# HaokunChen245/FedDAT

Measured on AMD Instinct MI355X. Metric: VQA samples/sec, ViLT-B/32 dual-adapter local step, higher is better.
Workload: dtype fp16; 1 GPU; configs[1] with fp16 operands (BASELINE.json's configs[1] string says bf16: same operand width and MFMA rate; the bf16 step is in other_operand_format with --full): ViLT-B/32 FedDAT, 1 client per MI355X, fp16 MFMA operands (dynamic loss scale, GradScaler semantics on the device, initial 2^14), fp32 accumulate / masters, batch=32/client, 384x384 synthetic + 40-token questions, MKD on; batch_per_client=32, seq_len=185, clients=1, hip_graph=True, ranks=1, hetero_steps=False

## Files before the change

### feddat_amd/csrc/head_tail.hip

```cpp
#include "common.hip.h"

namespace {

constexpr int HT_JT = 4;
constexpr int HT_NW = 8;
constexpr int HT_U = 3;

struct HtJob {
    const float* A; long sa_i, sa_k;
    const float* B; long sb_k, sb_j;
    int I, J, K;
    int mode;
    float alpha;
    const float* alpha_dev;
    const float* bias_j;
    float* out; long ldo;
    float* colsum;
    int pro;
    const float* pro_a;
    const float* pro_b;
    float pro_eps;
    float* stats_out;
    int epi;
    const float* aux; long ld_aux;
    int itiles, jblocks;
    int avec, bvec;
    int jt;
};
struct HtLaunch {
    HtJob job[2];
    int blocks0;
};

template <bool AV, bool BV, int JT>
__device__ __forceinline__ void ht_mainloop(const HtJob& p, const float* ap, const float* yp, const float* const (&bp)[JT],
                                            const bool iv, const bool (&jv)[JT], const int g, const float mean,
                                            const float rstd, const int c_first, const int c_step, f32x4 (&acc)[JT],
                                            float& asum) {
    const int nchunk = (p.K + 15) >> 4;
    for (int c0 = c_first; c0 < nchunk; c0 += c_step * HT_U) {
        f32x4 a[HT_U], y[HT_U], ga[HT_U], be[HT_U], b[HT_U][JT];
#pragma unroll
        for (int u = 0; u < HT_U; ++u) {
            const int k0 = (c0 + c_step * u) * 16 + 4 * g;
            const bool in = k0 < p.K;
            const int kc = in ? k0 : 0;
#pragma unroll
            for (int e = 0; e < 4; ++e) {
                const int ke = min(k0 + e, p.K - 1);
                if (!AV) a[u][e] = ap[(size_t)ke * p.sa_k];
                if (!AV && p.pro == FEDDAT_HT_PRO_TANH_BWD) y[u][e] = yp[(size_t)ke * p.sa_k];
            }
            if (AV) {
                a[u] = *reinterpret_cast<const f32x4*>(ap + kc);
                if (p.pro == FEDDAT_HT_PRO_TANH_BWD) y[u] = *reinterpret_cast<const f32x4*>(yp + kc);
            }
            if (p.pro == FEDDAT_HT_PRO_LN) {
                ga[u] = *reinterpret_cast<const f32x4*>(p.pro_a + kc);
                be[u] = *reinterpret_cast<const f32x4*>(p.pro_b + kc);
            }
#pragma unroll
            for (int t = 0; t < JT; ++t) {
                if (BV) {
                    b[u][t] = *reinterpret_cast<const f32x4*>(bp[t] + kc);
                } else {
#pragma unroll
                    for (int e = 0; e < 4; ++e) b[u][t][e] = bp[t][(size_t)min(k0 + e, p.K - 1) * p.sb_k];
                }
            }
        }
#pragma unroll
        for (int u = 0; u < HT_U; ++u) {
            const int k0 = (c0 + c_step * u) * 16 + 4 * g;
#pragma unroll
            for (int e = 0; e < 4; ++e) {
                const bool kv = (k0 + e) < p.K && (c0 + c_step * u) < nchunk;
                float av = a[u][e];
                if (p.pro == FEDDAT_HT_PRO_LN) av = (av - mean) * rstd * ga[u][e] + be[u][e];
                if (p.pro == FEDDAT_HT_PRO_TANH_BWD) av = av * (1.f - y[u][e] * y[u][e]);
                av = (iv && kv) ? av : 0.f;
                asum += av;
#pragma unroll
                for (int t = 0; t < JT; ++t) acc[t] = mfma16x4_f32(av, (jv[t] && kv) ? b[u][t][e] : 0.f, acc[t]);
            }
        }
    }
}

template <int JT>
__device__ __forceinline__ void ht_body(const HtJob& p, const int wid, float* ht_smem) {
    float (*red)[64][HT_JT * 4 + 4] = reinterpret_cast<float (*)[64][HT_JT * 4 + 4]>(ht_smem);
    float (*srow)[2] = reinterpret_cast<float (*)[2]>(ht_smem + (HT_NW - 1) * 64 * (HT_JT * 4 + 4));
    const int lane = threadIdx.x & 63, wave = threadIdx.x >> 6;
    const int itile = wid / p.jblocks, jb = wid - itile * p.jblocks;
    const int i16 = lane & 15, g = lane >> 4;
    const int i = itile * 16 + i16;
    const bool iv = i < p.I;
    const float* ap = p.A + (size_t)(iv ? i : 0) * p.sa_i;
    const float* yp = p.pro == FEDDAT_HT_PRO_TANH_BWD ? p.pro_a + (size_t)(iv ? i : 0) * p.sa_i : nullptr;

    float mean = 0.f, rstd = 0.f;
    if (p.pro == FEDDAT_HT_PRO_LN) {
        for (int rl = wave; rl < 16; rl += HT_NW) {
            const int r = itile * 16 + rl;
            if (r >= p.I) continue;
            const float* xr = p.A + (size_t)r * p.sa_i;
            const int nc = p.K >> 2;
            f32x4 v[8];
            float s = 0.f;
#pragma unroll
            for (int c = 0; c < 8; ++c) {
                const int q4 = lane + c * 64;
                if (q4 < nc) {
                    v[c] = *reinterpret_cast<const f32x4*>(xr + q4 * 4);
                    s += v[c][0] + v[c][1] + v[c][2] + v[c][3];
                }
            }
            const float m = wave_sum(s) / (float)p.K;
            float q = 0.f;
#pragma unroll
            for (int c = 0; c < 8; ++c)
                if (lane + c * 64 < nc)
#pragma unroll
                    for (int e = 0; e < 4; ++e) {
                        const float d = v[c][e] - m;
                        q += d * d;
                    }
            const float rs = rsqrtf(wave_sum(q) / (float)p.K + p.pro_eps);
            if (lane == 0) {
                srow[rl][0] = m;
                srow[rl][1] = rs;
                if (p.stats_out && jb == 0) {
                    p.stats_out[2 * r] = m;
                    p.stats_out[2 * r + 1] = rs;
                }
            }
        }
        __syncthreads();
        mean = srow[i16][0];
        rstd = srow[i16][1];
    }

    const int jgrp = p.mode == 0 ? jb : jb * HT_NW + wave;
    int j[JT];
    bool jv[JT];
    const float* bp[JT];
#pragma unroll
    for (int t = 0; t < JT; ++t) {
        j[t] = (jgrp * JT + t) * 16 + i16;
        jv[t] = j[t] < p.J;
        bp[t] = p.B + (size_t)(jv[t] ? j[t] : 0) * p.sb_j;
    }
    f32x4 acc[JT];
#pragma unroll
    for (int t = 0; t < JT; ++t) acc[t] = f32x4{0.f, 0.f, 0.f, 0.f};
    float asum = 0.f;
    const int c_first = p.mode == 0 ? wave : 0, c_step = p.mode == 0 ? HT_NW : 1;
    if (p.avec && p.bvec) ht_mainloop<true, true, JT>(p, ap, yp, bp, iv, jv, g, mean, rstd, c_first, c_step, acc, asum);
    else if (p.avec) ht_mainloop<true, false, JT>(p, ap, yp, bp, iv, jv, g, mean, rstd, c_first, c_step, acc, asum);
    else if (p.bvec) ht_mainloop<false, true, JT>(p, ap, yp, bp, iv, jv, g, mean, rstd, c_first, c_step, acc, asum);
    else ht_mainloop<false, false, JT>(p, ap, yp, bp, iv, jv, g, mean, rstd, c_first, c_step, acc, asum);
    asum += __shfl_xor(asum, 16, 64);
    asum += __shfl_xor(asum, 32, 64);
    if (p.mode == 0) {
        if (wave > 0) {
            float* dst = red[wave - 1][lane];
#pragma unroll
            for (int t = 0; t < JT; ++t) *reinterpret_cast<f32x4*>(dst + 4 * t) = acc[t];
            dst[JT * 4] = asum;
        }
        __syncthreads();
        if (wave != 0) return;
#pragma unroll 1
        for (int w = 0; w < HT_NW - 1; ++w) {
            const float* src = red[w][lane];
#pragma unroll
            for (int t = 0; t < JT; ++t) acc[t] = acc[t] + *reinterpret_cast<const f32x4*>(src + 4 * t);
            asum += src[JT * 4];
        }
    }
    const float alpha = p.alpha_dev ? p.alpha * *p.alpha_dev : p.alpha;
#pragma unroll
    for (int t = 0; t < JT; ++t) {
        if (!jv[t]) continue;
        const float bj = p.bias_j ? p.bias_j[j[t]] : 0.f;
#pragma unroll
        for (int e = 0; e < 4; ++e) {
            const int io = itile * 16 + 4 * g + e;
            if (io >= p.I) continue;
            float v = alpha * acc[t][e] + bj;
            if (p.epi == FEDDAT_HT_EPI_TANH) v = tanhf(v);
            if (p.epi == FEDDAT_HT_EPI_MUL_DGELU) v *= gelu_grad_f(p.aux[(size_t)io * p.ld_aux + j[t]]);
            p.out[(size_t)io * p.ldo + j[t]] = v;
        }
    }
    if (p.colsum && jgrp == 0 && g == 0 && iv) p.colsum[i] = alpha * asum;
}

__global__ __launch_bounds__(HT_NW * 64) void ht_gemm_kernel(const HtLaunch L) {
    extern __shared__ __attribute__((aligned(16))) float ht_smem[];
    const bool second = (int)blockIdx.x >= L.blocks0;
    const HtJob& p = L.job[second ? 1 : 0];
    const int wid = second ? blockIdx.x - L.blocks0 : blockIdx.x;
    if (p.jt == 1) ht_body<1>(p, wid, ht_smem);
    else ht_body<HT_JT>(p, wid, ht_smem);
}

__global__ __launch_bounds__(256) void ht_ln_gelu_kernel(const float* __restrict__ x, const float* __restrict__ gamma,
                                                         const float* __restrict__ beta, float eps, int rows, int H,
                                                         float* __restrict__ y, float* __restrict__ stats,
                                                         float* __restrict__ gl) {
    const int row = blockIdx.x * 4 + (threadIdx.x >> 6), lane = threadIdx.x & 63;
    if (row >= rows) return;
    const int nc = H >> 2;
    const float* xr = x + (size_t)row * H;
    f32x4 v[8];
    float s = 0.f;
#pragma unroll
    for (int c = 0; c < 8; ++c) {
        const int i = lane + c * 64;
        if (i < nc) {
            v[c] = *reinterpret_cast<const f32x4*>(xr + i * 4);
            s += v[c][0] + v[c][1] + v[c][2] + v[c][3];
        }
    }
    const float mean = wave_sum(s) / (float)H;
    float q = 0.f;
#pragma unroll
    for (int c = 0; c < 8; ++c)
        if (lane + c * 64 < nc)
#pragma unroll
            for (int e = 0; e < 4; ++e) {
                const float d = v[c][e] - mean;
                q += d * d;
            }
    const float rstd = rsqrtf(wave_sum(q) / (float)H + eps);
    if (lane == 0) {
        stats[2 * row] = mean;
        stats[2 * row + 1] = rstd;
    }
#pragma unroll
    for (int c = 0; c < 8; ++c) {
        const int i = lane + c * 64;
        if (i < nc) {
            const f32x4 g4 = *reinterpret_cast<const f32x4*>(gamma + i * 4);
// ... 492 lines not shown
__global__ void single_step_finish_kernel(const SingleFinish s, int* flag, float* scaler_f, int* scaler_i, float growth,
                                          float backoff, int growth_interval) {
    if (blockIdx.x != 0 || threadIdx.x != 0) return;
    const int applied = *flag ? 0 : 1;
    for (int k = 0; k < s.n; ++k) {
        s.state[k][0] += applied;
        s.state[k][1] += applied;
    }
    float scale = scaler_f[0];
    int tracker = scaler_i[0];
    if (!applied) {
        scale = fmaxf(scale * backoff, 6.103515625e-05f);
        tracker = 0;
        scaler_i[1] += 1;
        scaler_i[2] += 1;
    } else {
        tracker += 1;
        if (tracker >= growth_interval) {
            scale = fminf(scale * growth, 1073741824.0f);
            tracker = 0;
        }
    }
    scaler_f[0] = scale;
    scaler_f[1] = 1.0f / scale;
    scaler_i[0] = tracker;
    *flag = 0;
}

int ht_plan(const feddat_ht_job& s, feddat_ht_plan& p) {
    if (!(s.A && s.B && s.out && s.I > 0 && s.J > 0 && s.K > 0 && s.ldo >= s.J && (s.mode == 0 || s.mode == 1)))
        return FEDDAT_EINVAL;
    if (s.pro == FEDDAT_HT_PRO_LN && !(s.pro_a && s.pro_b && s.pro_eps > 0.f && s.sa_k == 1 && s.K % 4 == 0 && s.K <= 2048 &&
                                       s.sa_i % 4 == 0 && ((uintptr_t)s.A & 15) == 0))
        return FEDDAT_EINVAL;
    if (s.pro == FEDDAT_HT_PRO_TANH_BWD && !s.pro_a) return FEDDAT_EINVAL;
    if (s.epi == FEDDAT_HT_EPI_MUL_DGELU && !(s.aux && s.ld_aux >= s.J)) return FEDDAT_EINVAL;
    if (s.pro < 0 || s.pro > FEDDAT_HT_PRO_TANH_BWD || s.epi < 0 || s.epi > FEDDAT_HT_EPI_MUL_DGELU) return FEDDAT_EINVAL;
    p.avec = s.sa_k == 1 && s.K % 4 == 0 && s.sa_i % 4 == 0 && ((uintptr_t)s.A & 15) == 0 &&
             (s.pro != FEDDAT_HT_PRO_TANH_BWD || ((uintptr_t)s.pro_a & 15) == 0);
    p.bvec = s.sb_k == 1 && s.K % 4 == 0 && s.sb_j % 4 == 0 && ((uintptr_t)s.B & 15) == 0;
    if (s.pro == FEDDAT_HT_PRO_LN && !(p.avec && (((uintptr_t)s.pro_a | (uintptr_t)s.pro_b) & 15) == 0)) return FEDDAT_EINVAL;
    p.itiles = (s.I + 15) / 16;
    int jgroups = (s.J + 16 * HT_JT - 1) / (16 * HT_JT);
    p.jt = HT_JT;
    if (s.mode == 0 && p.itiles * jgroups < 64) {
        p.jt = 1;
        jgroups = (s.J + 15) / 16;
    }
    p.jblocks = s.mode == 0 ? jgroups : (jgroups + HT_NW - 1) / HT_NW;
    p.blocks = p.itiles * p.jblocks;
    return FEDDAT_OK;
}

int ht_fill(HtJob& j, const feddat_ht_job& s) {
    feddat_ht_plan p;
    const int rc = ht_plan(s, p);
    if (rc != FEDDAT_OK) return rc;
    j.A = s.A; j.sa_i = s.sa_i; j.sa_k = s.sa_k; j.B = s.B; j.sb_k = s.sb_k; j.sb_j = s.sb_j;
    j.I = s.I; j.J = s.J; j.K = s.K; j.mode = s.mode; j.alpha = s.alpha; j.alpha_dev = s.alpha_dev; j.bias_j = s.bias_j; j.out = s.out; j.ldo = s.ldo;
    j.colsum = s.colsum; j.pro = s.pro; j.pro_a = s.pro_a; j.pro_b = s.pro_b; j.pro_eps = s.pro_eps;
    j.stats_out = s.stats_out; j.epi = s.epi; j.aux = s.aux; j.ld_aux = s.ld_aux;
    j.avec = p.avec; j.bvec = p.bvec; j.jt = p.jt; j.itiles = p.itiles; j.jblocks = p.jblocks;
    return FEDDAT_OK;
}

}

extern "C" int feddat_head_gemm(const feddat_ht_job* jobs, int njobs, hipStream_t stream) {
    FD_CHECK_ARG(jobs && (njobs == 1 || njobs == 2));
    HtLaunch L{};
    int total = 0;
    for (int k = 0; k < njobs; ++k) {
        const int rc = ht_fill(L.job[k], jobs[k]);
        if (rc != FEDDAT_OK) return rc;
        const int nb = L.job[k].itiles * L.job[k].jblocks;
        if (k == 0) L.blocks0 = nb;
        total += nb;
    }
    constexpr int lds = ((HT_NW - 1) * 64 * (HT_JT * 4 + 4) + 32) * (int)sizeof(float);
    if (fd_set_max_lds((const void*)ht_gemm_kernel, lds) != FEDDAT_OK) return FEDDAT_ELAUNCH;
    hipLaunchKernelGGL(ht_gemm_kernel, dim3(total), dim3(HT_NW * 64), lds, stream, L);
    FD_LAUNCH_RET();
}

extern "C" int feddat_head_gemm_plan(const feddat_ht_job* job, feddat_ht_plan* out) {
    FD_CHECK_ARG(job && out);
    return ht_plan(*job, *out);
}

extern "C" int feddat_head_ln_gelu(const float* x, const float* gamma, const float* beta, float eps, int rows, int H,
                                   float* y, float* stats, float* gelu_out, hipStream_t stream) {
    FD_CHECK_ARG(x && gamma && beta && y && stats && gelu_out && rows > 0 && H > 0 && H % 4 == 0 && H <= 2048 && eps > 0.f);
    hipLaunchKernelGGL(ht_ln_gelu_kernel, dim3((rows + 3) / 4), dim3(256), 0, stream, x, gamma, beta, eps, rows, H, y, stats,
                       gelu_out);
    FD_LAUNCH_RET();
}

extern "C" int feddat_head_ln_bwd_full(const float* dy, const float* x, const float* stats, const float* gamma, int rows,
                                       int H, float* dx, float* dgamma, float* dbeta, hipStream_t stream) {
    FD_CHECK_ARG(dy && x && stats && gamma && dx && dgamma && dbeta && rows > 0 && rows <= 4096 && H > 0 && H % 4 == 0 &&
                 H <= 2048);
    hipLaunchKernelGGL(ht_ln_bwd_full_kernel, dim3((rows + 3) / 4 + (H + 63) / 64), dim3(256), 0, stream, dy, x, stats, gamma,
                       rows, H, dx, dgamma, dbeta);
    FD_LAUNCH_RET();
}

extern "C" int feddat_dat_loss_fwd_bwd_single(const float* logits, const float* teacher, const float* target, int B, int C,
                                              float temp, float* dlogits, float* scalars, hipStream_t stream) {
    FD_CHECK_ARG(logits && teacher && target && dlogits && scalars && B > 0 && B <= 4096 && C > 0 && C <= 128 && temp > 0.f);
    hipLaunchKernelGGL(dat_loss_single_kernel, dim3(1), dim3(1024), 2 * B * sizeof(float), stream, logits, teacher, target, B,
                       C, temp, dlogits, scalars, (int*)nullptr);
    FD_LAUNCH_RET();
}

extern "C" int feddat_dat_loss_fwd_bwd_checked(const float* logits, const float* teacher, const float* target, int B, int C,
                                               float temp, float* dlogits, float* scalars, int* nonfinite, hipStream_t stream) {
    FD_CHECK_ARG(logits && teacher && target && dlogits && scalars && B > 0 && B <= 4096 && C > 0 && C <= 128 && temp > 0.f);
    hipLaunchKernelGGL(dat_loss_single_kernel, dim3(1), dim3(1024), 2 * B * sizeof(float), stream, logits, teacher, target, B,
                       C, temp, dlogits, scalars, nonfinite);
    FD_LAUNCH_RET();
}

extern "C" int feddat_dat_loss_fwd_bwd_rows(const float* logits, const float* teacher, const float* target, int n, int B, int C,
                                            float temp, float* dlogits, float* scalars, int* nonfinite, hipStream_t stream) {
    FD_CHECK_ARG(logits && teacher && target && dlogits && scalars && n > 0 && n <= B && B <= 4096 && C > 0 && C <= 128 &&
                 temp > 0.f);
    hipLaunchKernelGGL(dat_loss_rows_kernel, dim3(1), dim3(1024), 2 * n * sizeof(float), stream, logits, teacher, target, n, B,
                       C, temp, dlogits, scalars, nonfinite);
    FD_LAUNCH_RET();
}

extern "C" long feddat_dat_loss_wide_workspace_elems(int B) { return B > 0 ? 2L * B : 0L; }

extern "C" int feddat_dat_loss_fwd_bwd_wide(const float* logits, const float* teacher, const float* target, int n, int B, int C,
                                            float temp, float* dlogits, float* scalars, int* nonfinite, float* workspace,
                                            long workspace_elems, hipStream_t stream) {
    FD_CHECK_ARG(logits && teacher && target && dlogits && scalars && workspace && n > 0 && n <= B && B <= 4096 && C > 0 &&
                 temp > 0.f && workspace_elems >= feddat_dat_loss_wide_workspace_elems(B));
    if (C <= WIDE_REG_C)
        hipLaunchKernelGGL(dat_loss_wide_kernel<true>, dim3(B), dim3(WIDE_T), 0, stream, logits, teacher, target, n, C, temp,
// ... 83 lines not shown
```

### feddat_amd/lib.py

```python
from __future__ import annotations

import contextlib
import ctypes as C
import os
import threading
from typing import Optional, Sequence

import torch

_PKG = os.path.dirname(os.path.abspath(__file__))
LIB_PATH = os.path.join(_PKG, "libfeddat_hip.so")
LIB_PATH_F16 = os.path.join(_PKG, "libfeddat_hip_f16.so")
OPERANDS_BF16, OPERANDS_FP16 = 0, 1
OPERAND_DTYPE = {"bf16": torch.bfloat16, "f16": torch.float16}

EPI_BF16, EPI_RESID_F32, EPI_GELU, EPI_MUL_DGELU, EPI_F32, EPI_GELU_G8, EPI_MUL_G8, EPI_GELU_G8_F8, EPI_MUL_G8_F8 = range(9)
F8_ACT_SCALE, F8_GRAD_HEADROOM = 0.125, 4.0
G8_LO, G8_STEP = -0.135, 0.005
GEMM_OP16, GEMM_FP8, GEMM_FP8MX = range(3)
GEMM_V1, GEMM_MID, GEMM_V2, GEMM_V3, GEMM_DUAL = range(5)

ABI_VERSION = 8
vp, i32, i64, f32, u32 = C.c_void_p, C.c_int, C.c_long, C.c_float, C.c_uint

# ... 89 lines not shown
    "feddat_layernorm_fwd_fp8": [vp, i64, vp, vp, f32, i32, i32, vp, vp, vp, vp, vp],
    "feddat_gemm_bf16_nt_skinny": [vp, i32, vp, i32, i32, i32, i32, i32, vp, vp, i32, vp, i32, vp, i32, vp, i32, vp, i32,
                                   vp, i64, vp],
    "feddat_attn_fwd": [vp, vp, vp, vp, i32, i32, i32, vp],
    "feddat_attn_bwd": [vp, vp, vp, vp, vp, vp, i32, i32, i32, vp],
    "feddat_attn_bwd_fp8mx": [vp, vp, vp, vp, vp, vp, vp, i32, i32, i32, vp],
    "feddat_attn_cls_fwd": [vp, vp, vp, vp, i32, i32, i32, vp],
    "feddat_attn_cls_bwd": [vp, vp, vp, vp, vp, vp, i32, i32, i32, vp],
    "feddat_attn2_fwd": [vp, i64, vp, i64, vp, i64, vp, i32, vp, i64, vp, i32, i32, i32, i64, i64, i32, vp],
    "feddat_attn2_bwd": [vp, i64, vp, i64, vp, i64, vp, i32, vp, i64, vp, vp, i64, vp, vp, i64, vp, i64, vp, i64, i32, i32,
                         i32, i64, i64, i32, vp],
    "feddat_attn2_fwd_dropout": [vp, i64, vp, i64, vp, i64, vp, i32, vp, i64, vp, i32, i32, i32, i64, i64, i32, f32, u32, u32,
                                 vp, vp],
    "feddat_attn2_bwd_dropout": [vp, i64, vp, i64, vp, i64, vp, i32, vp, i64, vp, vp, i64, vp, vp, i64, vp, i64, vp, i64,
                                 i32, i32, i32, i64, i64, i32, f32, u32, u32, vp, vp],
    "feddat_dropout": [vp, vp, vp, vp, vp, i64, f32, u32, u32, vp, vp],
    "feddat_layernorm_fwd": [vp, i64, vp, vp, f32, i32, i32, vp, vp, vp, vp],
    "feddat_layernorm_bwd_dx": [vp, vp, i64, vp, i64, vp, vp, vp, i64, i32, i32, vp, i64, vp, vp],
    "feddat_layernorm_bwd_dx_sparse": [vp, vp, i64, vp, i64, vp, vp, vp, i64, i32, i32, i32, vp, i64, vp, vp],
    "feddat_layernorm_bwd_full": [vp, vp, vp, vp, i32, i32, vp, vp, vp, vp],
    "feddat_adapter_fwd": [vp, vp, i32, i32, i32, C.POINTER(AdapterSeg), i32, vp, vp],
    "feddat_adapter_fwd_ln": [vp, vp, i32, i32, i32, C.POINTER(AdapterSeg), i32, vp, vp, f32, vp, vp, vp, vp],
    "feddat_adapter_bwd": [vp, vp, vp, vp, vp, vp, vp, i32, i32, i32, C.POINTER(AdapterSeg), i32, vp],
    "feddat_adapter_bwd_fp8": [vp, vp, vp, vp, vp, vp, vp, i32, i32, i32, C.POINTER(AdapterSeg), i32, vp],
    "feddat_adapter_pack": [vp, vp, vp, vp, vp, vp, i32, i32, vp],
    "feddat_adapter_pack_strided": [vp, vp, i64, vp, vp, vp, vp, i64, i32, i32, i32, vp],
    "feddat_adapter_wgrad_workspace_elems": [i32],
    "feddat_adapter_wgrad": [C.POINTER(WgradSeg), i32, vp, i64, i32, i32, vp],
    "feddat_adapter_wgrad_partial": [C.POINTER(WgradSeg), i32, vp, i64, i32, i32, vp],
    "feddat_adapter_wgrad_reduce": [vp, i32, i32, vp, i64, vp],
    "feddat_adapter_wgrad_reduce_checked": [vp, i32, i32, vp, i64, vp, vp],
    "feddat_vilt_layer_fwd": [vp, C.POINTER(ViltLayerWeights), C.POINTER(ViltLayerActs), i32, i32, i32, vp, i32,
                              C.POINTER(AdapterSeg), i32, vp, vp, vp],
    "feddat_vilt_layer_bwd": [vp, C.POINTER(ViltLayerWeights), C.POINTER(ViltLayerActs), C.POINTER(ViltLayerGrads), i32, i32,
                              i32, vp, C.POINTER(AdapterSeg), i32, C.POINTER(WgradSeg), i32, vp, i64, i32, vp],
    "feddat_sgemm_f32": [vp, i64, i64, vp, i64, i64, i32, i32, i32, i32, f32, vp, vp, i64, i64, vp, i64, vp],
    "feddat_reduce_partials": [vp, i64, i32, i64, vp, vp],
    "feddat_dat_loss_fwd_bwd": [vp, vp, vp, i32, i32, f32, vp, vp, vp],
    "feddat_dat_loss_fwd_bwd_single": [vp, vp, vp, i32, i32, f32, vp, vp, vp],
    "feddat_dat_loss_fwd_bwd_checked": [vp, vp, vp, i32, i32, f32, vp, vp, vp, vp],
    "feddat_dat_step_finish": [vp, vp, vp, vp, vp, vp, f32, f32, i32, vp],
    "feddat_bce_loss_fwd_bwd": [vp, vp, i32, i32, vp, vp, vp, vp],
    "feddat_single_step_finish": [C.POINTER(vp), i32, vp, vp, vp, f32, f32, i32, vp],
    "feddat_dat_loss_fwd_bwd_rows": [vp, vp, vp, i32, i32, i32, f32, vp, vp, vp, vp],
    "feddat_bce_loss_fwd_bwd_rows": [vp, vp, i32, i32, i32, vp, vp, vp, vp],
    "feddat_dat_loss_wide_workspace_elems": [i32],
    "feddat_dat_loss_fwd_bwd_wide": [vp, vp, vp, i32, i32, i32, f32, vp, vp, vp, vp, i64, vp],
    "feddat_vector_grad_workspace_elems": [i32, i32],
    "feddat_colsum_partial": [vp, vp, i64, vp, i32, i32, vp, i64, vp],
    "feddat_ln_param_grad_partial": [vp, vp, i64, vp, i64, vp, i32, i32, vp, vp, i64, vp],
    "feddat_vector_grad_reduce": [vp, i32, i32, f32, vp, vp, vp],
    "feddat_head_gemm": [C.POINTER(HtJob), i32, vp],
    "feddat_head_gemm_plan": [C.POINTER(HtJob), C.POINTER(HtPlan)],
    "feddat_head_ln_gelu": [vp, vp, vp, f32, i32, i32, vp, vp, vp, vp],
    "feddat_head_ln_bwd_full": [vp, vp, vp, vp, i32, i32, vp, vp, vp, vp],
    "feddat_adamw_multi": [C.POINTER(AdamwGroup), i32, f32, i32, i32, f32, f32, f32, vp],
    "feddat_step_tick_multi": [C.POINTER(vp), C.POINTER(i32), C.POINTER(i32), i32, vp],
    "feddat_vqa_score_accumulate": [vp, vp, i32, i32, vp, vp],
    "feddat_lm_loss_fwd_bwd": [vp, vp, i64, vp, vp, vp, i32, i32, f32, f32, f32, vp, i64, vp, vp],
    "feddat_lm_loss_fwd_bwd_dyn": [vp, vp, i64, vp, vp, vp, i32, i32, f32, f32, f32, vp, vp, vp, i64, vp, vp],
    "feddat_axpby3": [vp, f32, vp, f32, vp, f32, vp, vp, i64, vp],
    "feddat_vilt_stage_inputs": [vp, vp, vp, vp, vp, vp, vp, vp, vp, vp, i32, i32, i32, i32, i32, i32, vp],
    "feddat_vilt_pad_batch": [vp, vp, vp, vp, vp, vp, i32, i32, i32, i32, i32, i32, vp],
    "feddat_softmax_gather_rows": [vp, i64, i32, i32, vp, i64, i32, vp, vp],
    "feddat_topk_rows": [vp, i64, vp, i32, i32, i32, i32, vp, vp, vp],
    "feddat_albef_pad_questions": [vp, vp, vp, i32, i32, i64, i32, vp],
    "feddat_rank_slab_gather": [vp, vp, vp, vp, vp, vp, vp, vp, i32, i32, i32, i32, i32, i32, i32, i32, i64, vp],
    "feddat_rank_slab_loss": [vp, vp, i32, i32, i32, i32, i32, i32, vp],
    "feddat_gather_rows": [vp, vp, vp, vp, i32, i32, vp],
    "feddat_segment_sum_rows": [vp, vp, vp, i32, i32, i32, vp],
    "feddat_adamw_flat": [vp, vp, vp, vp, i64, vp, vp, i32, vp, f32, i32, i32, f32, f32, f32, vp],
    "feddat_step_tick": [vp, i32, i32, vp],
    "feddat_text_embed": [vp, vp, vp, vp, vp, vp, vp, f32, vp, vp, i32, i32, i32, i32, vp],
    "feddat_im2col_patches": [vp, vp, i32, i32, i32, i32, i32, vp],
    "feddat_image_embed_assemble": [vp, vp, vp, vp, i64, vp, vp, i32, i32, i32, i32, i32, vp],
    "feddat_image_embed_assemble_masked": [vp, vp, vp, vp, vp, vp, vp, vp, vp, i32, i32, i32, i32, i32, i32, i32, vp],
    "feddat_im2col_patches_slots": [vp, vp, vp, i32, i32, i32, i32, i32, i32, i32, vp],
    "feddat_image_embed_assemble_slots": [vp, vp, vp, vp, vp, vp, vp, vp, vp, vp, i32, i32, i32, i32, i32, i32, i32, i32, vp],
    "feddat_pos_embed_resize_masked": [vp, vp, vp, i32, i32, i32, i32, i32, i32, vp],
    "feddat_vilt_key_mask": [vp, vp, vp, i32, i32, i32, i32, i32, i32, vp],
    "feddat_vilt_image_workspace_bytes": [vp, vp, vp, vp, i32],
    "feddat_vilt_image_preprocess": [vp, vp, vp, vp, vp, vp, i32, i32, i32, vp, vp, vp, i64, vp],
    "feddat_pos_embed_resize": [vp, vp, i32, i32, i32, i32, vp],
    "feddat_wordpiece_table_entries": [i32],
    "feddat_wordpiece_table_build": [vp, vp, i32, vp, i64],
    "feddat_wordpiece_encode": [vp, vp, i32, vp, i64, i32, i32, i32, i32, i32, vp, vp, vp, vp],
    "feddat_cvt_f32_bf16": [vp, vp, i64, vp],
    "feddat_transpose_f32_bf16": [vp, vp, i32, i32, vp],
    "feddat_tanh_fwd": [vp, i64, vp],
    "feddat_tanh_bwd": [vp, vp, vp, i64, vp],
    "feddat_gelu_fwd": [vp, vp, i64, vp],
    "feddat_gelu_bwd": [vp, vp, vp, i64, vp],
    "feddat_scatter_cls_rows": [vp, vp, vp, i32, i32, i32, vp],
    "feddat_fedavg_accumulate": [vp, vp, i64, f32, f32, i32, vp],
    "feddat_probe_tr16": [vp, vp, vp],
}

EXPORTED_SYMBOLS = tuple(_SIGS.keys())


class FeddatHipError(RuntimeError):
    pass


_lib = None
_lib_f16 = None
# ... 408 lines not shown
         "feddat_adapter_pack")


def vilt_layer_fwd(ctx: "Context", W, A, nb, S, heads, segs_arr, *, key_mask=None, ln1_done=False, next_ln_g=None,
                   next_ln_b=None):
    _chk(load().feddat_vilt_layer_fwd(ctx._h, C.byref(W), C.byref(A), nb, S, heads, _p(key_mask), int(ln1_done), segs_arr,
                                      len(segs_arr), _p(next_ln_g), _p(next_ln_b), _stream()), "feddat_vilt_layer_fwd")


def vilt_layer_bwd(ctx: "Context", W, A, G, nb, S, heads, segs_arr, wsegs_arr, partials, *, key_mask=None,
                   wgrad_reduce_now=True):
    _chk(load().feddat_vilt_layer_bwd(ctx._h, C.byref(W), C.byref(A), C.byref(G), nb, S, heads, _p(key_mask), segs_arr,
                                      len(segs_arr), wsegs_arr, 0 if wsegs_arr is None else len(wsegs_arr), _p(partials),
                                      0 if partials is None else partials.numel(), int(wgrad_reduce_now), _stream()),
         "feddat_vilt_layer_bwd")


def sgemm_f32(A, sa_i, sa_k, B, sb_k, sb_j, I, J, K, out, *, ldo=None, ksplit=1, alpha=1.0, bias_j=None,
              out_split_stride=0, colsum=None, colsum_split_stride=None):
    _dev(A, B, out)
    _chk(load().feddat_sgemm_f32(_p(A), sa_i, sa_k, _p(B), sb_k, sb_j, I, J, K, ksplit, alpha, _p(bias_j), _p(out),
                                 J if ldo is None else ldo, out_split_stride, _p(colsum),
                                 I if colsum_split_stride is None else colsum_split_stride, _stream()),
         "feddat_sgemm_f32")


def reduce_partials(inp, stride, nsplit, n, out):
    _dev(inp, out)
    _chk(load().feddat_reduce_partials(_p(inp), stride, nsplit, n, _p(out), _stream()), "feddat_reduce_partials")


def dat_loss_fwd_bwd(logits, teacher, target, dlogits, scalars, temp=3.0):
    _dev(logits, teacher, target)
    B, Cn = logits.shape
    assert scalars.numel() >= 4 + 2 * B
    _chk(load().feddat_dat_loss_fwd_bwd(_p(logits), _p(teacher), _p(target), B, Cn, temp, _p(dlogits), _p(scalars),
                                        _stream()), "feddat_dat_loss_fwd_bwd")


def ht_job(A, sa_i, sa_k, B, sb_k, sb_j, I, J, K, out, ldo=None, mode=0, alpha=1.0, bias_j=None, colsum=None, pro=HT_PRO_NONE,
           pro_a=None, pro_b=None, pro_eps=0.0, stats_out=None, epi=HT_EPI_NONE, aux=None, ld_aux=0, alpha_dev=None) -> HtJob:
    _dev(A, B, out)
    j = HtJob()
    j._keep = (A, B, out, bias_j, colsum, pro_a, pro_b, stats_out, aux, alpha_dev)
    ptr = lambda t: t.data_ptr() if t is not None else None
    j.A, j.sa_i, j.sa_k, j.B, j.sb_k, j.sb_j = ptr(A), sa_i, sa_k, ptr(B), sb_k, sb_j
    j.I, j.J, j.K, j.mode, j.alpha = I, J, K, mode, alpha
    j.bias_j, j.out, j.ldo, j.colsum = ptr(bias_j), ptr(out), (J if ldo is None else ldo), ptr(colsum)
    j.pro, j.pro_a, j.pro_b, j.pro_eps, j.stats_out = pro, ptr(pro_a), ptr(pro_b), pro_eps, ptr(stats_out)
    j.epi, j.aux, j.ld_aux, j.alpha_dev = epi, ptr(aux), ld_aux, ptr(alpha_dev)
    return j


def head_gemm(*jobs: HtJob):
    arr = (HtJob * len(jobs))(*jobs)
    arr._keep = jobs
    _chk(load().feddat_head_gemm(arr, len(jobs), _stream()), "feddat_head_gemm")


def head_gemm_plan(job: HtJob) -> dict:
    p = HtPlan()
    _chk(load().feddat_head_gemm_plan(C.byref(job), C.byref(p)), "feddat_head_gemm_plan")
    return {n: getattr(p, n) for n, _ in HtPlan._fields_}


def head_ln_gelu(x, gamma, beta, eps, y, stats, gelu_out):
    _dev(x, y, stats, gelu_out)
    _chk(load().feddat_head_ln_gelu(_p(x), _p(gamma), _p(beta), eps, x.shape[0], x.shape[1], _p(y), _p(stats), _p(gelu_out),
                                    _stream()), "feddat_head_ln_gelu")


def head_ln_bwd_full(dy, x, stats, gamma, dx, dgamma, dbeta):
    _dev(dy, x, stats, dx)
    _chk(load().feddat_head_ln_bwd_full(_p(dy), _p(x), _p(stats), _p(gamma), x.shape[0], x.shape[1], _p(dx), _p(dgamma),
                                        _p(dbeta), _stream()), "feddat_head_ln_bwd_full")


def dat_loss_fwd_bwd_single(logits, teacher, target, dlogits, scalars, temp=3.0):
    _dev(logits, teacher, target)
    B, Cn = logits.shape
    assert scalars.numel() >= 4
    _chk(load().feddat_dat_loss_fwd_bwd_single(_p(logits), _p(teacher), _p(target), B, Cn, temp, _p(dlogits), _p(scalars),
                                               _stream()), "feddat_dat_loss_fwd_bwd_single")


def dat_loss_fwd_bwd_checked(logits, teacher, target, dlogits, scalars, nonfinite, temp=3.0):
    _dev(logits, teacher, target, nonfinite)
    B, Cn = logits.shape
    assert scalars.numel() >= 4 and nonfinite.dtype == torch.int32
    _chk(load().feddat_dat_loss_fwd_bwd_checked(_p(logits), _p(teacher), _p(target), B, Cn, temp, _p(dlogits), _p(scalars),
                                                _p(nonfinite), _stream()), "feddat_dat_loss_fwd_bwd_checked")


def dat_step_finish(head_state, ad1_state, ad0_state, flags, scaler_f, scaler_i, growth=2.0, backoff=0.5, growth_interval=2000):
    _dev(head_state, ad1_state, ad0_state, flags, scaler_f, scaler_i)
    _chk(load().feddat_dat_step_finish(_p(head_state), _p(ad1_state), _p(ad0_state), _p(flags), _p(scaler_f), _p(scaler_i),
                                       growth, backoff, growth_interval, _stream()), "feddat_dat_step_finish")


def bce_loss_fwd_bwd(logits, target, dlogits, scalars, nonfinite=None):
    _dev(logits, target, dlogits, scalars)
    B, Cn = logits.shape
    assert scalars.numel() >= 1 and (nonfinite is None or nonfinite.dtype == torch.int32)
    _chk(load().feddat_bce_loss_fwd_bwd(_p(logits), _p(target), B, Cn, _p(dlogits), _p(scalars),
                                        _p(nonfinite), _stream()), "feddat_bce_loss_fwd_bwd")


def dat_loss_fwd_bwd_rows(logits, teacher, target, dlogits, scalars, n, nonfinite=None, temp=3.0):
    _dev(logits, teacher, target, dlogits, scalars, nonfinite)
    B, Cn = dlogits.shape
    assert scalars.numel() >= 4 and (nonfinite is None or nonfinite.dtype == torch.int32)
    assert logits.shape[0] >= n and teacher.shape[0] >= n and target.shape[0] >= n and logits.shape[1] == Cn
    _chk(load().feddat_dat_loss_fwd_bwd_rows(_p(logits), _p(teacher), _p(target), int(n), B, Cn, temp, _p(dlogits), _p(scalars),
                                             _p(nonfinite), _stream()), "feddat_dat_loss_fwd_bwd_rows")


# ... 386 lines not shown
```

### include/feddat_hip.h

```cpp
#ifndef FEDDAT_HIP_H
#define FEDDAT_HIP_H

#include <stdint.h>

#ifdef __cplusplus
extern "C" {
#endif

#ifndef __HIP__
typedef struct ihipStream_t* hipStream_t;
#endif

#define FEDDAT_OK 0
#define FEDDAT_EINVAL 1
#define FEDDAT_ELAUNCH 2
#define FEDDAT_ETIMEOUT 3

#define FEDDAT_ABI_VERSION 8
int feddat_abi_version(void);
#define FEDDAT_OPERANDS_BF16 0
#define FEDDAT_OPERANDS_FP16 1
int feddat_operand_format(void);

typedef struct feddat_ctx feddat_ctx;
// ... 169 lines not shown
    float* st1_next;
} feddat_vilt_layer_acts;
typedef struct {
    float* dh_out;
    float* dh_in;
    float* dh3;
    void* dh16;
    void* dU;
    void* dx16;
    void* dctx;
    void* dqkv;
    float* z;
    float* dz;
} feddat_vilt_layer_grads;
int feddat_vilt_layer_fwd(feddat_ctx* ctx, const feddat_vilt_layer_weights* W, const feddat_vilt_layer_acts* A, int nb,
                          int S, int heads, const uint8_t* key_mask, int ln1_done, const feddat_adapter_seg* segs, int nseg,
                          const float* next_ln_g, const float* next_ln_b, hipStream_t stream);
int feddat_vilt_layer_bwd(feddat_ctx* ctx, const feddat_vilt_layer_weights* W, const feddat_vilt_layer_acts* A,
                          const feddat_vilt_layer_grads* G, int nb, int S, int heads, const uint8_t* key_mask,
                          const feddat_adapter_seg* segs, int nseg, const feddat_wgrad_seg* wsegs, int nwseg,
                          float* wgrad_partials, long wgrad_partials_elems, int wgrad_reduce_now, hipStream_t stream);

int feddat_sgemm_f32(const float* A, long sa_i, long sa_k, const float* B, long sb_k, long sb_j, int I, int J, int K,
                     int ksplit, float alpha, const float* bias_j, float* out, long ldo, long out_split_stride,
                     float* colsum, long colsum_split_stride, hipStream_t stream);
int feddat_reduce_partials(const float* in, long stride, int nsplit, long n, float* out, hipStream_t stream);

#define FEDDAT_HT_PRO_NONE 0
#define FEDDAT_HT_PRO_LN 1
#define FEDDAT_HT_PRO_TANH_BWD 2
#define FEDDAT_HT_EPI_NONE 0
#define FEDDAT_HT_EPI_TANH 1
#define FEDDAT_HT_EPI_MUL_DGELU 2
typedef struct feddat_ht_job {
    const float* A; long sa_i, sa_k;
    const float* B; long sb_k, sb_j;
    int I, J, K, mode;
    float alpha;
    const float* bias_j;
    float* out; long ldo;
    float* colsum;
    int pro;
    const float* pro_a; const float* pro_b; float pro_eps;
    float* stats_out;
    int epi;
    const float* aux; long ld_aux;
    const float* alpha_dev;
} feddat_ht_job;
int feddat_head_gemm(const feddat_ht_job* jobs, int njobs, hipStream_t stream);
typedef struct feddat_ht_plan {
    int avec, bvec, jt, itiles, jblocks, blocks;
} feddat_ht_plan;
int feddat_head_gemm_plan(const feddat_ht_job* job, feddat_ht_plan* out);
int feddat_head_ln_gelu(const float* x, const float* gamma, const float* beta, float eps, int rows, int H, float* y,
                        float* stats, float* gelu_out, hipStream_t stream);
int feddat_head_ln_bwd_full(const float* dy, const float* x, const float* stats, const float* gamma, int rows, int H,
                            float* dx, float* dgamma, float* dbeta, hipStream_t stream);
int feddat_dat_loss_fwd_bwd_single(const float* logits, const float* teacher, const float* target, int B, int C, float temp,
                                   float* dlogits, float* scalars, hipStream_t stream);
int feddat_dat_loss_fwd_bwd_checked(const float* logits, const float* teacher, const float* target, int B, int C, float temp,
                                    float* dlogits, float* scalars, int* nonfinite, hipStream_t stream);
#define FEDDAT_ADAMW_MAX_GROUPS 4
typedef struct feddat_adamw_group {
    float* p; const float* g; float* m; float* v; long n;
    const long* seg_off; const float* seg_wd; int nseg;
    const int* state; int d_sched, d_adam;
    const int* skip_if[2];
    float* bak; int bak_mode;
    const int* restore_if;
} feddat_adamw_group;
int feddat_adamw_multi(const feddat_adamw_group* groups, int ngroups, float base_lr, int warmup, int total, float beta1,
                       float beta2, float eps, hipStream_t stream);
int feddat_step_tick_multi(int* const* states, const int* d_sched, const int* d_adam, int n, hipStream_t stream);
int feddat_dat_step_finish(int* head_state, int* ad1_state, int* ad0_state, int* flags, float* scaler_f, int* scaler_i,
                           float growth, float backoff, int growth_interval, hipStream_t stream);
int feddat_bce_loss_fwd_bwd(const float* logits, const float* target, int B, int C, float* dlogits, float* scalars,
                            int* nonfinite, hipStream_t stream);
int feddat_single_step_finish(int* const* states, int n, int* flag, float* scaler_f, int* scaler_i, float growth,
                              float backoff, int growth_interval, hipStream_t stream);
int feddat_dat_loss_fwd_bwd_rows(const float* logits, const float* teacher, const float* target, int n, int B, int C, float temp,
                                 float* dlogits, float* scalars, int* nonfinite, hipStream_t stream);
int feddat_bce_loss_fwd_bwd_rows(const float* logits, const float* target, int n, int B, int C, float* dlogits, float* scalars,
                                 int* nonfinite, hipStream_t stream);
long feddat_dat_loss_wide_workspace_elems(int B);
int feddat_dat_loss_fwd_bwd_wide(const float* logits, const float* teacher, const float* target, int n, int B, int C, float temp,
                                 float* dlogits, float* scalars, int* nonfinite, float* workspace, long workspace_elems,
                                 hipStream_t stream);

typedef struct feddat_vgrad_job {
    const float* partials;
    float* grad;
    int slabs;
    int n;
    int flags;
    int reserved;
} feddat_vgrad_job;
#define FEDDAT_VGRAD_UNSCALED 1
long feddat_vector_grad_workspace_elems(int rows, int N);
int feddat_colsum_partial(const void* x_bf16, const float* x_f32, long x_stride, const unsigned char* row_mask, int rows,
                          int N, float* partials, long partials_elems, hipStream_t stream);
int feddat_ln_param_grad_partial(const void* dy_bf16, const float* dy_f32, long dy_stride, const float* x, long x_stride,
                                 const float* stats, int rows, int N, float* dgamma_partials, float* dbeta_partials,
                                 long partials_elems, hipStream_t stream);
int feddat_vector_grad_reduce(const feddat_vgrad_job* jobs_dev, int njobs, int max_n, float unscale,
                              const float* unscale_dev, int* nonfinite, hipStream_t stream);

// ... 105 lines not shown
```

Measured before the change: 4568 samples/s.

## Software-pipeline head GEMM mainloop with deeper register prefetch

Adds a deep mainloop for the head/tail split-K GEMM that loads the next batch of 6 or 12 K-chunks into registers while the current batch is multiplied. For the LayerNorm prologue it issues the first loads before computing row statistics, so that latency is hidden. Epilogue bias and aux loads are also hoisted ahead of the cross-wave reduction. The depth is picked automatically from K per wave; the cost is higher register pressure and possibly lower occupancy, and explicit fmaf with contraction turned off keeps the numerics fixed.

Result: no change. 4568 samples/s (median of 3 runs) (+0.0%).

```diff
diff --git a/feddat_amd/csrc/head_tail.hip b/feddat_amd/csrc/head_tail.hip
--- a/feddat_amd/csrc/head_tail.hip
+++ b/feddat_amd/csrc/head_tail.hip
@@ -5,6 +5,8 @@
 constexpr int HT_JT = 4;
 constexpr int HT_NW = 8;
 constexpr int HT_U = 3;
+constexpr int HT_UD = 6;
+constexpr int HT_UDD = 12;
 
 struct HtJob {
     const float* A; long sa_i, sa_k;
@@ -26,11 +28,73 @@
     int itiles, jblocks;
     int avec, bvec;
     int jt;
+    int depth;
 };
 struct HtLaunch {
     HtJob job[2];
     int blocks0;
 };
+
+template <int JT, int U>
+struct HtRegs {
+    f32x4 a[U], y[U], ga[U], be[U], b[U][JT];
+};
+
+template <bool AV, bool BV, int JT, int U, bool PRO = true>
+__device__ __forceinline__ void ht_load(const HtJob& p, const float* ap, const float* yp, const float* const (&bp)[JT],
+                                        const int g, const int c0, const int c_step, HtRegs<JT, U>& r) {
+#pragma unroll
+    for (int u = 0; u < U; ++u) {
+        const int k0 = (c0 + c_step * u) * 16 + 4 * g;
+        const bool in = k0 < p.K;
+        const int kc = in ? k0 : 0;
+#pragma unroll
+        for (int e = 0; e < 4; ++e) {
+            const int ke = min(k0 + e, p.K - 1);
+            if (!AV) r.a[u][e] = ap[(size_t)ke * p.sa_k];
+            if (PRO && !AV && p.pro == FEDDAT_HT_PRO_TANH_BWD) r.y[u][e] = yp[(size_t)ke * p.sa_k];
+        }
+        if (AV) {
+            r.a[u] = *reinterpret_cast<const f32x4*>(ap + kc);
+            if (PRO && p.pro == FEDDAT_HT_PRO_TANH_BWD) r.y[u] = *reinterpret_cast<const f32x4*>(yp + kc);
+        }
+        if (PRO && p.pro == FEDDAT_HT_PRO_LN) {
+            r.ga[u] = *reinterpret_cast<const f32x4*>(p.pro_a + kc);
+            r.be[u] = *reinterpret_cast<const f32x4*>(p.pro_b + kc);
+        }
+#pragma unroll
+        for (int t = 0; t < JT; ++t) {
+            if (BV) {
+                r.b[u][t] = *reinterpret_cast<const f32x4*>(bp[t] + kc);
+            } else {
+#pragma unroll
+                for (int e = 0; e < 4; ++e) r.b[u][t][e] = bp[t][(size_t)min(k0 + e, p.K - 1) * p.sb_k];
+            }
+        }
+    }
+}
+
+template <int JT, int U, bool PRO = true>
+__device__ __forceinline__ void ht_mma(const HtJob& p, const HtRegs<JT, U>& r, const bool iv, const bool (&jv)[JT], const int g,
+                                       const float mean, const float rstd, const int c0, const int c_step, const int nchunk,
+                                       f32x4 (&acc)[JT], float& asum) {
+#pragma unroll
+    for (int u = 0; u < U; ++u) {
+        const int k0 = (c0 + c_step * u) * 16 + 4 * g;
+#pragma unroll
+        for (int e = 0; e < 4; ++e) {
+#pragma clang fp contract(off)
+            const bool kv = (k0 + e) < p.K && (c0 + c_step * u) < nchunk;
+            float av = r.a[u][e];
+            if (PRO && p.pro == FEDDAT_HT_PRO_LN) av = __builtin_fmaf((av - mean) * rstd, r.ga[u][e], r.be[u][e]);
+            if (PRO && p.pro == FEDDAT_HT_PRO_TANH_BWD) av = av * __builtin_fmaf(-r.y[u][e], r.y[u][e], 1.f);
+            av = (iv && kv) ? av : 0.f;
+            asum += av;
+#pragma unroll
+            for (int t = 0; t < JT; ++t) acc[t] = mfma16x4_f32(av, (jv[t] && kv) ? r.b[u][t][e] : 0.f, acc[t]);
+        }
+    }
+}
 
 template <bool AV, bool BV, int JT>
 __device__ __forceinline__ void ht_mainloop(const HtJob& p, const float* ap, const float* yp, const float* const (&bp)[JT],
@@ -39,51 +103,75 @@
                                             float& asum) {
     const int nchunk = (p.K + 15) >> 4;
     for (int c0 = c_first; c0 < nchunk; c0 += c_step * HT_U) {
-        f32x4 a[HT_U], y[HT_U], ga[HT_U], be[HT_U], b[HT_U][JT];
-#pragma unroll
-        for (int u = 0; u < HT_U; ++u) {
-            const int k0 = (c0 + c_step * u) * 16 + 4 * g;
-            const bool in = k0 < p.K;
-            const int kc = in ? k0 : 0;
-#pragma unroll
-            for (int e = 0; e < 4; ++e) {
-                const int ke = min(k0 + e, p.K - 1);
-                if (!AV) a[u][e] = ap[(size_t)ke * p.sa_k];
-                if (!AV && p.pro == FEDDAT_HT_PRO_TANH_BWD) y[u][e] = yp[(size_t)ke * p.sa_k];
-            }
-            if (AV) {
-                a[u] = *reinterpret_cast<const f32x4*>(ap + kc);
-                if (p.pro == FEDDAT_HT_PRO_TANH_BWD) y[u] = *reinterpret_cast<const f32x4*>(yp + kc);
-            }
-            if (p.pro == FEDDAT_HT_PRO_LN) {
-                ga[u] = *reinterpret_cast<const f32x4*>(p.pro_a + kc);
-                be[u] = *reinterpret_cast<const f32x4*>(p.pro_b + kc);
-            }
-#pragma unroll
-            for (int t = 0; t < JT; ++t) {
-                if (BV) {
-                    b[u][t] = *reinterpret_cast<const f32x4*>(bp[t] + kc);
+        HtRegs<JT, HT_U> r;
+        ht_load<AV, BV, JT, HT_U>(p, ap, yp, bp, g, c0, c_step, r);
+        ht_mma<JT, HT_U>(p, r, iv, jv, g, mean, rstd, c0, c_step, nchunk, acc, asum);
+    }
+}
+
+__device__ __forceinline__ void ht_ln_stats(const HtJob& p, const int itile, const int jb, float (*srow)[2], float& mean,
+                                            float& rstd) {
+    const int lane = threadIdx.x & 63, wave = threadIdx.x >> 6;
+    for (int rl = wave; rl < 16; rl += HT_NW) {
+        const int r = itile * 16 + rl;
+        if (r >= p.I) continue;
+        const float* xr = p.A + (size_t)r * p.sa_i;
+        const int nc = p.K >> 2;
+        f32x4 v[8];
+        float s = 0.f;
+#pragma unroll
+        for (int c = 0; c < 8; ++c) {
+            const int q4 = lane + c * 64;
+            if (q4 < nc) {
+                v[c] = *reinterpret_cast<const f32x4*>(xr + q4 * 4);
+                s += v[c][0] + v[c][1] + v[c][2] + v[c][3];
+            }
+        }
+        const float m = wave_sum(s) / (float)p.K;
+        float q = 0.f;
+#pragma unroll
+        for (int c = 0; c < 8; ++c)
+            if (lane + c * 64 < nc) {
+#pragma clang fp contract(off)
+                const float d0 = v[c][0] - m, d1 = v[c][1] - m, d2 = v[c][2] - m, d3 = v[c][3] - m;
+                if (c == 0) {
+                    q = d3 * d3 + __builtin_fmaf(d2, d2, __builtin_fmaf(d0, d0, d1 * d1));
                 } else {
-#pragma unroll
-                    for (int e = 0; e < 4; ++e) b[u][t][e] = bp[t][(size_t)min(k0 + e, p.K - 1) * p.sb_k];
+                    q += d0 * d0;
+                    q += d1 * d1;
+                    q += d2 * d2;
+                    q += d3 * d3;
                 }
             }
-        }
-#pragma unroll
-        for (int u = 0; u < HT_U; ++u) {
-            const int k0 = (c0 + c_step * u) * 16 + 4 * g;
-#pragma unroll
-            for (int e = 0; e < 4; ++e) {
-                const bool kv = (k0 + e) < p.K && (c0 + c_step * u) < nchunk;
-                float av = a[u][e];
-                if (p.pro == FEDDAT_HT_PRO_LN) av = (av - mean) * rstd * ga[u][e] + be[u][e];
-                if (p.pro == FEDDAT_HT_PRO_TANH_BWD) av = av * (1.f - y[u][e] * y[u][e]);
-                av = (iv && kv) ? av : 0.f;
-                asum += av;
-#pragma unroll
-                for (int t = 0; t < JT; ++t) acc[t] = mfma16x4_f32(av, (jv[t] && kv) ? b[u][t][e] : 0.f, acc[t]);
-            }
-        }
+        const float rs = rsqrtf(wave_sum(q) / (float)p.K + p.pro_eps);
+        if (lane == 0) {
+            srow[rl][0] = m;
+            srow[rl][1] = rs;
+            if (p.stats_out && jb == 0) {
+                p.stats_out[2 * r] = m;
+                p.stats_out[2 * r + 1] = rs;
+            }
+        }
+    }
+    __syncthreads();
+    mean = srow[lane & 15][0];
+    rstd = srow[lane & 15][1];
+}
+
+template <int JT, int U>
+__device__ __forceinline__ void ht_deep(const HtJob& p, const float* ap, const float* yp, const float* const (&bp)[JT],
+                                        const bool iv, const bool (&jv)[JT], const int g, const int itile, const int jb,
+                                        float (*srow)[2], const int c_first, const int c_step, f32x4 (&acc)[JT], float& asum) {
+    constexpr bool PRO = JT == 1 && U == HT_UD;
+    const int nchunk = (p.K + 15) >> 4;
+    HtRegs<JT, U> r;
+    if (c_first < nchunk) ht_load<true, true, JT, U, PRO>(p, ap, yp, bp, g, c_first, c_step, r);
+    float mean = 0.f, rstd = 0.f;
+    if (PRO && p.pro == FEDDAT_HT_PRO_LN) ht_ln_stats(p, itile, jb, srow, mean, rstd);
+    for (int c0 = c_first; c0 < nchunk;) {
+        ht_mma<JT, U, PRO>(p, r, iv, jv, g, mean, rstd, c0, c_step, nchunk, acc, asum);
+        c0 += c_step * U;
+        if (c0 < nchunk) ht_load<true, true, JT, U, PRO>(p, ap, yp, bp, g, c0, c_step, r);
     }
 }
 
@@ -99,48 +187,6 @@
     const float* ap = p.A + (size_t)(iv ? i : 0) * p.sa_i;
     const float* yp = p.pro == FEDDAT_HT_PRO_TANH_BWD ? p.pro_a + (size_t)(iv ? i : 0) * p.sa_i : nullptr;
 
-    float mean = 0.f, rstd = 0.f;
-    if (p.pro == FEDDAT_HT_PRO_LN) {
-        for (int rl = wave; rl < 16; rl += HT_NW) {
-            const int r = itile * 16 + rl;
-            if (r >= p.I) continue;
-            const float* xr = p.A + (size_t)r * p.sa_i;
-            const int nc = p.K >> 2;
-            f32x4 v[8];
-            float s = 0.f;
-#pragma unroll
-            for (int c = 0; c < 8; ++c) {
-                const int q4 = lane + c * 64;
-                if (q4 < nc) {
-                    v[c] = *reinterpret_cast<const f32x4*>(xr + q4 * 4);
-                    s += v[c][0] + v[c][1] + v[c][2] + v[c][3];
-                }
-            }
-            const float m = wave_sum(s) / (float)p.K;
-            float q = 0.f;
-#pragma unroll
-            for (int c = 0; c < 8; ++c)
-                if (lane + c * 64 < nc)
-#pragma unroll
-                    for (int e = 0; e < 4; ++e) {
-                        const float d = v[c][e] - m;
-                        q += d * d;
-                    }
-            const float rs = rsqrtf(wave_sum(q) / (float)p.K + p.pro_eps);
-            if (lane == 0) {
-                srow[rl][0] = m;
-                srow[rl][1] = rs;
-                if (p.stats_out && jb == 0) {
-                    p.stats_out[2 * r] = m;
-                    p.stats_out[2 * r + 1] = rs;
-                }
-            }
-        }
-        __syncthreads();
-        mean = srow[i16][0];
-        rstd = srow[i16][1];
-    }
-
     const int jgrp = p.mode == 0 ? jb : jb * HT_NW + wave;
     int j[JT];
     bool jv[JT];
@@ -156,10 +202,33 @@
     for (int t = 0; t < JT; ++t) acc[t] = f32x4{0.f, 0.f, 0.f, 0.f};
     float asum = 0.f;
     const int c_first = p.mode == 0 ? wave : 0, c_step = p.mode == 0 ? HT_NW : 1;
-    if (p.avec && p.bvec) ht_mainloop<true, true, JT>(p, ap, yp, bp, iv, jv, g, mean, rstd, c_first, c_step, acc, asum);
-    else if (p.avec) ht_mainloop<true, false, JT>(p, ap, yp, bp, iv, jv, g, mean, rstd, c_first, c_step, acc, asum);
-    else if (p.bvec) ht_mainloop<false, true, JT>(p, ap, yp, bp, iv, jv, g, mean, rstd, c_first, c_step, acc, asum);
-    else ht_mainloop<false, false, JT>(p, ap, yp, bp, iv, jv, g, mean, rstd, c_first, c_step, acc, asum);
+    if (p.depth == HT_UD) {
+        ht_deep<JT, HT_UD>(p, ap, yp, bp, iv, jv, g, itile, jb, srow, c_first, c_step, acc, asum);
+    } else if (JT == 1 && p.depth == HT_UDD) {
+        ht_deep<JT, (JT == 1 ? HT_UDD : HT_UD)>(p, ap, yp, bp, iv, jv, g, itile, jb, srow, c_first, c_step, acc, asum);
+    } else {
+        float mean = 0.f, rstd = 0.f;
+        if (p.pro == FEDDAT_HT_PRO_LN) ht_ln_stats(p, itile, jb, srow, mean, rstd);
+        if (p.avec && p.bvec) ht_mainloop<true, true, JT>(p, ap, yp, bp, iv, jv, g, mean, rstd, c_first, c_step, acc, asum);
+        else if (p.avec) ht_mainloop<true, false, JT>(p, ap, yp, bp, iv, jv, g, mean, rstd, c_first, c_step, acc, asum);
+        else if (p.bvec) ht_mainloop<false, true, JT>(p, ap, yp, bp, iv, jv, g, mean, rstd, c_first, c_step, acc, asum);
+        else ht_mainloop<false, false, JT>(p, ap, yp, bp, iv, jv, g, mean, rstd, c_first, c_step, acc, asum);
+    }
+    const bool writer = p.mode != 0 || wave == 0;
+    float alpha = p.alpha, bj[JT];
+    f32x4 ax[JT];
+    if (writer) {
+        if (p.alpha_dev) alpha = p.alpha * *p.alpha_dev;
+#pragma unroll
+        for (int t = 0; t < JT; ++t) {
+            bj[t] = (jv[t] && p.bias_j) ? p.bias_j[j[t]] : 0.f;
+#pragma unroll
+            for (int e = 0; e < 4; ++e) {
+                const int io = itile * 16 + 4 * g + e;
+                ax[t][e] = (p.epi == FEDDAT_HT_EPI_MUL_DGELU && jv[t] && io < p.I) ? p.aux[(size_t)io * p.ld_aux + j[t]] : 0.f;
+            }
+        }
+    }
     asum += __shfl_xor(asum, 16, 64);
     asum += __shfl_xor(asum, 32, 64);
     if (p.mode == 0) {
@@ -179,18 +248,16 @@
             asum += src[JT * 4];
         }
     }
-    const float alpha = p.alpha_dev ? p.alpha * *p.alpha_dev : p.alpha;
 #pragma unroll
     for (int t = 0; t < JT; ++t) {
         if (!jv[t]) continue;
-        const float bj = p.bias_j ? p.bias_j[j[t]] : 0.f;
 #pragma unroll
         for (int e = 0; e < 4; ++e) {
             const int io = itile * 16 + 4 * g + e;
             if (io >= p.I) continue;
-            float v = alpha * acc[t][e] + bj;
+            float v = __builtin_fmaf(alpha, acc[t][e], bj[t]);
             if (p.epi == FEDDAT_HT_EPI_TANH) v = tanhf(v);
-            if (p.epi == FEDDAT_HT_EPI_MUL_DGELU) v *= gelu_grad_f(p.aux[(size_t)io * p.ld_aux + j[t]]);
+            if (p.epi == FEDDAT_HT_EPI_MUL_DGELU) v *= gelu_grad_f(ax[t][e]);
             p.out[(size_t)io * p.ldo + j[t]] = v;
         }
     }
@@ -789,10 +856,26 @@
     return FEDDAT_OK;
 }
 
-int ht_fill(HtJob& j, const feddat_ht_job& s) {
+bool ht_depth_ok(const feddat_ht_job& s, const feddat_ht_plan& p, const int depth) {
+    if (depth == HT_U) return true;
+    if (!(p.avec && p.bvec)) return false;
+    if (depth == HT_UD) return p.jt == 1 || s.pro == FEDDAT_HT_PRO_NONE;
+    return depth == HT_UDD && p.jt == 1 && s.pro == FEDDAT_HT_PRO_NONE;
+}
+
+int ht_depth(const feddat_ht_job& s, const feddat_ht_plan& p) {
+    const int per_wave = ((s.K + 15) / 16 + HT_NW - 1) / HT_NW;
+    if (s.mode != 0 || per_wave <= HT_U) return HT_U;
+    if (per_wave > HT_UD && ht_depth_ok(s, p, HT_UDD)) return HT_UDD;
+    return ht_depth_ok(s, p, HT_UD) ? HT_UD : HT_U;
+}
+
+int ht_fill(HtJob& j, const feddat_ht_job& s, const int depth) {
     feddat_ht_plan p;
     const int rc = ht_plan(s, p);
     if (rc != FEDDAT_OK) return rc;
+    if (depth != 0 && !ht_depth_ok(s, p, depth)) return FEDDAT_EINVAL;
+    j.depth = depth ? depth : ht_depth(s, p);
     j.A = s.A; j.sa_i = s.sa_i; j.sa_k = s.sa_k; j.B = s.B; j.sb_k = s.sb_k; j.sb_j = s.sb_j;
     j.I = s.I; j.J = s.J; j.K = s.K; j.mode = s.mode; j.alpha = s.alpha; j.alpha_dev = s.alpha_dev; j.bias_j = s.bias_j; j.out = s.out; j.ldo = s.ldo;
     j.colsum = s.colsum; j.pro = s.pro; j.pro_a = s.pro_a; j.pro_b = s.pro_b; j.pro_eps = s.pro_eps;
@@ -803,12 +886,12 @@
 
 }
 
-extern "C" int feddat_head_gemm(const feddat_ht_job* jobs, int njobs, hipStream_t stream) {
+extern "C" int feddat_head_gemm_depth(const feddat_ht_job* jobs, int njobs, int depth, hipStream_t stream) {
     FD_CHECK_ARG(jobs && (njobs == 1 || njobs == 2));
     HtLaunch L{};
     int total = 0;
     for (int k = 0; k < njobs; ++k) {
-        const int rc = ht_fill(L.job[k], jobs[k]);
+        const int rc = ht_fill(L.job[k], jobs[k], depth);
         if (rc != FEDDAT_OK) return rc;
         const int nb = L.job[k].itiles * L.job[k].jblocks;
         if (k == 0) L.blocks0 = nb;
@@ -820,9 +903,20 @@
     FD_LAUNCH_RET();
 }
 
+extern "C" int feddat_head_gemm(const feddat_ht_job* jobs, int njobs, hipStream_t stream) {
+    return feddat_head_gemm_depth(jobs, njobs, 0, stream);
+}
+
 extern "C" int feddat_head_gemm_plan(const feddat_ht_job* job, feddat_ht_plan* out) {
     FD_CHECK_ARG(job && out);
     return ht_plan(*job, *out);
+}
+
+extern "C" int feddat_head_gemm_plan_depth(const feddat_ht_job* job, feddat_ht_plan* out, int* depth) {
+    FD_CHECK_ARG(job && out && depth);
+    const int rc = ht_plan(*job, *out);
+    if (rc == FEDDAT_OK) *depth = ht_depth(*job, *out);
+    return rc;
 }
 
 extern "C" int feddat_head_ln_gelu(const float* x, const float* gamma, const float* beta, float eps, int rows, int H,
diff --git a/feddat_amd/lib.py b/feddat_amd/lib.py
--- a/feddat_amd/lib.py
+++ b/feddat_amd/lib.py
@@ -165,6 +165,8 @@
     "feddat_vector_grad_reduce": [vp, i32, i32, f32, vp, vp, vp],
     "feddat_head_gemm": [C.POINTER(HtJob), i32, vp],
     "feddat_head_gemm_plan": [C.POINTER(HtJob), C.POINTER(HtPlan)],
+    "feddat_head_gemm_plan_depth": [C.POINTER(HtJob), C.POINTER(HtPlan), C.POINTER(C.c_int)],
+    "feddat_head_gemm_depth": [C.POINTER(HtJob), i32, i32, vp],
     "feddat_head_ln_gelu": [vp, vp, vp, f32, i32, i32, vp, vp, vp, vp],
     "feddat_head_ln_bwd_full": [vp, vp, vp, vp, i32, i32, vp, vp, vp, vp],
     "feddat_adamw_multi": [C.POINTER(AdamwGroup), i32, f32, i32, i32, f32, f32, f32, vp],
@@ -679,9 +681,25 @@
     return j
 
 
+_ht_shallow = False
+
+
+@contextlib.contextmanager
+def head_gemm_shallow():
+    global _ht_shallow
+    prev, _ht_shallow = _ht_shallow, True
+    try:
+        yield
+    finally:
+        _ht_shallow = prev
+
+
 def head_gemm(*jobs: HtJob):
     arr = (HtJob * len(jobs))(*jobs)
     arr._keep = jobs
+    if _ht_shallow:
+        _chk(load().feddat_head_gemm_depth(arr, len(jobs), 3, _stream()), "feddat_head_gemm_depth")
+        return
     _chk(load().feddat_head_gemm(arr, len(jobs), _stream()), "feddat_head_gemm")
 
 
@@ -689,6 +707,18 @@
     p = HtPlan()
     _chk(load().feddat_head_gemm_plan(C.byref(job), C.byref(p)), "feddat_head_gemm_plan")
     return {n: getattr(p, n) for n, _ in HtPlan._fields_}
+
+
+def head_gemm_depth(depth: int, *jobs: HtJob):
+    arr = (HtJob * len(jobs))(*jobs)
+    arr._keep = jobs
+    _chk(load().feddat_head_gemm_depth(arr, len(jobs), depth, _stream()), "feddat_head_gemm_depth")
+
+
+def head_gemm_plan_depth(job: HtJob) -> dict:
+    p, d = HtPlan(), C.c_int(0)
+    _chk(load().feddat_head_gemm_plan_depth(C.byref(job), C.byref(p), C.byref(d)), "feddat_head_gemm_plan_depth")
+    return dict({n: getattr(p, n) for n, _ in HtPlan._fields_}, depth=d.value)
 
 
 def head_ln_gelu(x, gamma, beta, eps, y, stats, gelu_out):
diff --git a/include/feddat_hip.h b/include/feddat_hip.h
--- a/include/feddat_hip.h
+++ b/include/feddat_hip.h
@@ -245,6 +245,8 @@
     int avec, bvec, jt, itiles, jblocks, blocks;
 } feddat_ht_plan;
 int feddat_head_gemm_plan(const feddat_ht_job* job, feddat_ht_plan* out);
+int feddat_head_gemm_plan_depth(const feddat_ht_job* job, feddat_ht_plan* out, int* depth);
+int feddat_head_gemm_depth(const feddat_ht_job* jobs, int njobs, int depth, hipStream_t stream);
 int feddat_head_ln_gelu(const float* x, const float* gamma, const float* beta, float eps, int rows, int H, float* y,
                         float* stats, float* gelu_out, hipStream_t stream);
 int feddat_head_ln_bwd_full(const float* dy, const float* x, const float* stats, const float* gamma, int rows, int H,
```
